# HIPS/DESI-MCMC

Hardware: AMD Instinct MI355X
Metric: source-pixel evals/sec + full-field log-lik ms, 10k sources x 5 bands x 2048^2 (higher is better)
Workload: dtype f64

## Files before the change

desi-mcmc_amd/csrc/k_render_hw.h:

```cpp
#pragma once
#include "k_render.h"

#ifdef CEL_ABLATE
#define CEL_ABLATE_BITS(flags) ((flags) >> 8)
#else
#define CEL_ABLATE_BITS(flags) 0
#endif

#define HW_TW 32
#define HW_TH 64
#ifdef HW_SYNC_BARRIER
#define HW_WAVE_SYNC() __syncthreads()
#else
#define HW_WAVE_SYNC()                                              \
    do {                                                            \
        __builtin_amdgcn_fence(__ATOMIC_ACQ_REL, "wavefront");      \
        __builtin_amdgcn_wave_barrier();                            \
    } while (0)
#endif
#define HW_PAD 12
#ifndef HW_PART_ENTRIES
#define HW_PART_ENTRIES 12
#endif

__host__ __device__ inline double quad_max_rect_hw(double a, double b, double c, double x1, double x2, double y1, double y2) {
    double m = a * x1 * x1 + (2.0 * b * x1 + c * y1) * y1;
    m = fmax(m, a * x2 * x2 + (2.0 * b * x2 + c * y1) * y1);
    m = fmax(m, a * x1 * x1 + (2.0 * b * x1 + c * y2) * y2);
    m = fmax(m, a * x2 * x2 + (2.0 * b * x2 + c * y2) * y2);
    return m * 1.00001;
}

template <int G, int STRIDE = HW_TW, bool SUM = false>
__device__ inline void rec_group_hw(const CompTab &T, const double *__restrict__ et, int k0, double x,
                                    int Y0, int ra, int rb, int L, bool on, double *__restrict__ acc_col,
                                    double *__restrict__ msum = nullptr) {
    double g[G], r[G], q[G];
    const double aon = on ? 1.0 : 0.0;
    for (int sa = ra; sa < rb; sa += L) {
        const int sb = min(sa + L, rb);
        const double y0 = (double)(Y0 + sa);
#pragma unroll
        for (int i = 0; i < G; i++) {
            const int k = k0 + i;
            double dx = x - T.mx[k], dy = y0 - T.my[k];
            double qb = T.qb[k], qc = T.qc[k];
            double hx = qb * dx + qc * dy;
            double e = -0.5 * (T.qa[k] * dx * dx + (qb * dx + hx) * dy);
            double er = fmin(fmax(-(hx + 0.5 * qc), -REC_EMAX * EXP_SCALE), REC_EMAX * EXP_SCALE);
            g[i] = (T.A[k] * aon) * exp_tab64(e, et);
            r[i] = exp_tab64(er, et);
            q[i] = T.eq[k];
        }
        int row = sa;
        for (; row + 1 < sb; row += 2) {
#pragma clang fp contract(off)
            double s0 = g[0], s1, g1[G], r1[G];
#pragma unroll
            for (int i = 1; i < G; i++) s0 += g[i];
#pragma unroll
            for (int i = 0; i < G; i++) {
                g1[i] = g[i] * r[i];
                r1[i] = r[i] * q[i];
            }
            s1 = g1[0];
#pragma unroll
            for (int i = 1; i < G; i++) s1 += g1[i];
#pragma unroll
            for (int i = 0; i < G; i++) {
                g[i] = g1[i] * r1[i];
                r[i] = r1[i] * q[i];
            }
            if (SUM) { *msum += s0; *msum += s1; }
            else {
                lds_add(&acc_col[row * STRIDE], s0);
                lds_add(&acc_col[(row + 1) * STRIDE], s1);
            }
        }
        if (row < sb) {
            double s0 = g[0];
#pragma unroll
            for (int i = 1; i < G; i++) s0 += g[i];
            if (SUM) *msum += s0;
            else lds_add(&acc_col[row * STRIDE], s0);
        }
    }
}

template <int N, int NT>
__device__ __forceinline__ void rec_walk_n(double (&g)[NT], double (&r)[NT], const double (&q)[NT], int row, int rend, bool advance,
                                           double *__restrict__ acc_col) {
    for (; row + 1 < rend; row += 2) {
#pragma clang fp contract(off)
        double s0 = g[0], s1, g1[N], r1[N];
#pragma unroll
        for (int i = 1; i < N; i++) s0 += g[i];
#pragma unroll
        for (int i = 0; i < N; i++) {
            g1[i] = g[i] * r[i];
            r1[i] = r[i] * q[i];
        }
        s1 = g1[0];
#pragma unroll
        for (int i = 1; i < N; i++) s1 += g1[i];
#pragma unroll
        for (int i = 0; i < N; i++) {
            g[i] = g1[i] * r1[i];
            r[i] = r1[i] * q[i];
        }
        lds_add(&acc_col[row * HW_TW], s0);
        lds_add(&acc_col[(row + 1) * HW_TW], s1);
    }
    if (row < rend) {
#pragma clang fp contract(off)
        double s0 = g[0];
#pragma unroll
        for (int i = 1; i < N; i++) s0 += g[i];
        lds_add(&acc_col[row * HW_TW], s0);
        if (advance) {
#pragma unroll
            for (int i = 0; i < N; i++) {
                g[i] = g[i] * r[i];
                r[i] = r[i] * q[i];
            }
        }
    }
}

template <int NB, int NS>
__device__ inline void rec_group_nested(const CompTab &T, const double *__restrict__ et, int kb, int ks, double x, int Y0,
                                        int ga, int gb, int sa, int sb, bool on, double *__restrict__ acc_col) {
    constexpr int NT = NB + NS;
    double g[NT], r[NT], q[NT];
    const double aon = on ? 1.0 : 0.0;
    auto seed = [&](int i, int k, double y0) {
        double dx = x - T.mx[k], dy = y0 - T.my[k];
        double qb = T.qb[k], qc = T.qc[k];
        double hx = qb * dx + qc * dy;
        double e = -0.5 * (T.qa[k] * dx * dx + (qb * dx + hx) * dy);
        double er = fmin(fmax(-(hx + 0.5 * qc), -REC_EMAX * EXP_SCALE), REC_EMAX * EXP_SCALE);
        g[i] = (T.A[k] * aon) * exp_tab64(e, et);
        r[i] = exp_tab64(er, et);
        q[i] = T.eq[k];
    };
#pragma unroll
    for (int i = 0; i < NB; i++) seed(i, kb + i, (double)(Y0 + ga));
    rec_walk_n<NB, NT>(g, r, q, ga, sa, true, acc_col);
#pragma unroll
    for (int i = 0; i < NS; i++) seed(NB + i, ks + i, (double)(Y0 + sa));
    rec_walk_n<NT, NT>(g, r, q, sa, sb, true, acc_col);
    rec_walk_n<NB, NT>(g, r, q, sb, gb, false, acc_col);
}

__host__ __device__ inline int nested_big(int gA) { return gA >= 5 ? 3 : (gA == 4 ? 2 : gA); }

template <int SHIFT = 3>
__device__ __forceinline__ int slot_by_rows(bool keep, int rlo, int rhi) {
    const int cls = keep ? 7 - min((rhi - rlo - 1) >> SHIFT, 7) : 8;
    int slot = 0, base = 0;
#pragma unroll
    for (int q = 0; q < 8; q++) {
        const unsigned long long bq = __ballot(cls == q);
        const int within = __builtin_amdgcn_mbcnt_hi((unsigned)(bq >> 32), __builtin_amdgcn_mbcnt_lo((unsigned)bq, 0));
        if (cls == q) slot = base + within;
        base += __popcll(bq);
    }
    return slot;
}

struct StarTab {
    double px[64], py[64], scale[64];
    int4 box[64];
    int cum[64];
    double qa[K_PSF], qb[K_PSF], qc[K_PSF], eq[K_PSF], A0[K_PSF], mux[K_PSF], muy[K_PSF];
};
static_assert(sizeof(StarTab) <= sizeof(CompTab), "the star table must fit the component table's storage");
#define STAR_EMAX 600.0


__device__ __forceinline__ bool star_setup(StarTab &ST, const BandDev *__restrict__ bd, const double *__restrict__ et, int lane) {
    bool bad = false;
    if (lane < K_PSF) {
        const double cxx = bd->cxx[lane], cxy = bd->cxy[lane], cyy = bd->cyy[lane];
        const double inv = 1.0 / (cxx * cyy - cxy * cxy);
        const double qa = cyy * inv, qb = -cxy * inv, qc = cxx * inv;
        ST.qa[lane] = qa * EXP_SCALE; ST.qb[lane] = qb * EXP_SCALE; ST.qc[lane] = qc * EXP_SCALE;
        ST.eq[lane] = exp_tab64(-qc * EXP_SCALE, et);
        ST.A0[lane] = bd->w[lane] * (0.5 / PI_D) * sqrt(inv);
        ST.mux[lane] = bd->mux[lane]; ST.muy[lane] = bd->muy[lane];
        const double rb_ = bd->R + 2.0;
        const double emax = 0.5 * quad_max_rect_hw(qa, qb, qc, -rb_ - bd->mux[lane], rb_ - bd->mux[lane],
                                                   -rb_ - bd->muy[lane], rb_ - bd->muy[lane]);
        bad = !(emax <= STAR_EMAX);
    }
    const bool ok = (__ballot(bad) == 0ull);
    __syncthreads();
    return ok;
}

__device__ __forceinline__ void star_stage(const RenderArgs &a, StarTab &ST, const SrcRec *__restrict__ recs, int64_t off, int base, int nb,
                                           int lane, int X0, int Y0, int strict, int lfirst = 0, int lstride = 1 ) {
    __syncthreads();
    double2 pp = make_double2(0.0, 0.0);
    double sc = 0.0;
    int4 bx4 = make_int4(0, 0, 0, 0);
    int nrows = -1;
    if (lane < nb) {
        const SrcRec *rp = recs + a.lists[off + lfirst + (int64_t)lstride * (base + lane)];
        pp = *reinterpret_cast<const double2 *>(&rp->px);
        sc = rp->scale;
        bx4 = *reinterpret_cast<const int4 *>(&rp->x0);
        nrows = max(min(bx4.w, Y0 + HW_TH) - max(bx4.z + strict, Y0), 0);
        const int ncols = max(min(bx4.y, X0 + HW_TW) - max(bx4.x + strict, X0), 0);
        if (ncols == 0) nrows = 0;
    }
    int *srows = reinterpret_cast<int *>(ST.scale);
    srows[lane] = nrows;
    __syncthreads();
    int rank = 0;
    for (int j = 0; j < nb; j++) {
        const int rj = srows[j];
        rank += (rj > nrows || (rj == nrows && j < lane)) ? 1 : 0;
    }
    __syncthreads();
    if (lane < nb) {
        ST.px[rank] = pp.x; ST.py[rank] = pp.y; ST.scale[rank] = sc;
        ST.box[rank] = bx4;
    }
    __syncthreads();
}

template <bool DIAG, int CW>
__device__ __forceinline__ void star_walk(const RenderArgs &a, StarTab &ST, const double *__restrict__ et, double *__restrict__ acc,
                                          int nb, int lane, int Xa, int Y0, int strict, unsigned &dbg_halfrows,
                                          unsigned char *__restrict__ own = nullptr) {
    double cqa[K_PSF], cqb[K_PSF], cqc[K_PSF], ceq[K_PSF], cA0[K_PSF], cmx[K_PSF], cmy[K_PSF];
#pragma unroll
    for (int k = 0; k < K_PSF; k++) {
        cqa[k] = ST.qa[k]; cqb[k] = ST.qb[k]; cqc[k] = ST.qc[k]; ceq[k] = ST.eq[k];
        cA0[k] = ST.A0[k]; cmx[k] = ST.mux[k]; cmy[k] = ST.muy[k];
    }
    const int dbg = DIAG ? CEL_ABLATE_BITS(a.flags) : 0;
    int w = 0;
    if (lane < nb) {
        const int4 q = ST.box[lane];
        const int nr = max(min(q.w, Y0 + HW_TH) - max(q.z + strict, Y0), 0);
        w = (nr > 0) ? max(min(q.y, Xa + CW) - max(q.x + strict, Xa), 0) : 0;
    }
    int incl = w;
#pragma unroll
    for (int o = 1; o < 64; o <<= 1) {
        const int up = __shfl_up(incl, o);
        if (lane >= o) incl += up;
    }
    const int total = __builtin_amdgcn_readlane(incl, 63);
    ST.cum[lane] = (lane < nb) ? incl - w : 0x3fffffff;
    if (own) {
#pragma unroll
        for (int cidx = 0; cidx < CW; cidx++)
            if (cidx < w) own[incl - w + cidx] = (unsigned char)lane;
    }
    __syncthreads();
    for (int t0 = 0; t0 < total && !(dbg & 2); t0 += 64) {
        const int t = t0 + lane;
        const bool valid = t < total;
        int j = 0;
        if (own) {
            j = own[min(t, total - 1)];
        } else {
#pragma unroll
            for (int step = 32; step > 0; step >>= 1)
                if (ST.cum[min(j + step, 63)] <= t && j + step < 64) j += step;
        }
        const double px = ST.px[j], py = ST.py[j];
        const int4 bx = ST.box[j];
        const int bx0 = max(bx.x + strict, Xa), by0 = bx.z + strict;
        const int xi = bx0 + (t - ST.cum[j]);
        const int ra = max(by0, Y0) - Y0;
        const int n = (valid && !(dbg & 1)) ? max(min(bx.w, Y0 + HW_TH) - Y0 - ra, 0) : 0;
        const double amp = valid ? ST.scale[j] : 0.0;
        const int nmax = __builtin_amdgcn_readlane(n, 0);
        if (DIAG && a.timing) dbg_halfrows += 2u * (unsigned)nmax * K_PSF;
        const double x = (double)xi;
        double g[K_PSF], r[K_PSF];
        const double y0 = (double)(Y0 + ra);
#pragma unroll
        for (int k = 0; k < K_PSF; k++) {
            const double dx = x - (px + cmx[k]), dy = y0 - (py + cmy[k]);
            const double hx = cqb[k] * dx + cqc[k] * dy;
            const double e = -0.5 * (cqa[k] * dx * dx + (cqb[k] * dx + hx) * dy);
            const double er = fmin(fmax(-(hx + 0.5 * cqc[k]), -REC_EMAX * EXP_SCALE), REC_EMAX * EXP_SCALE);
            g[k] = (cA0[k] * amp) * exp_tab64(e, et);
            r[k] = exp_tab64(er, et);
        }
        double *rowp = acc + ra * CW + (valid ? xi - Xa : 0);
        int i = 0;
        for (; i + 3 < nmax; i += 4, rowp += 4 * CW) {
#pragma clang fp contract(off)
            double g1[K_PSF], r1[K_PSF];
            const double s0 = (g[0] + g[1]) + g[2];
#pragma unroll
            for (int k = 0; k < K_PSF; k++) { g1[k] = g[k] * r[k]; r1[k] = r[k] * ceq[k]; }
            const double s1 = (g1[0] + g1[1]) + g1[2];
#pragma unroll
            for (int k = 0; k < K_PSF; k++) { g[k] = g1[k] * r1[k]; r[k] = r1[k] * ceq[k]; }
            const double s2 = (g[0] + g[1]) + g[2];
#pragma unroll
            for (int k = 0; k < K_PSF; k++) { g1[k] = g[k] * r[k]; r1[k] = r[k] * ceq[k]; }
            const double s3 = (g1[0] + g1[1]) + g1[2];
#pragma unroll
            for (int k = 0; k < K_PSF; k++) { g[k] = g1[k] * r1[k]; r[k] = r1[k] * ceq[k]; }
            if (i + 3 < n) {
                lds_add(&rowp[0], s0);
                lds_add(&rowp[CW], s1);
                lds_add(&rowp[2 * CW], s2);
                lds_add(&rowp[3 * CW], s3);
            } else {
                if (i < n) lds_add(&rowp[0], s0);
                if (i + 1 < n) lds_add(&rowp[CW], s1);
                if (i + 2 < n) lds_add(&rowp[2 * CW], s2);
            }
        }
        for (; i < nmax; i++, rowp += CW) {
#pragma clang fp contract(off)
            if (i < n) lds_add(&rowp[0], (g[0] + g[1]) + g[2]);
#pragma unroll
            for (int k = 0; k < K_PSF; k++) { g[k] = g[k] * r[k]; r[k] = r[k] * ceq[k]; }
        }
    }
}

template <bool DIAG>
__device__ __forceinline__ void star_pass(const RenderArgs &a, StarTab &ST, const double *__restrict__ et, double *__restrict__ acc,
                                          const SrcRec *__restrict__ recs, int64_t off, int nstar, int lane, int X0, int Y0,
                                          int strict, unsigned &dbg_halfrows, unsigned &dbg_pairs, int lfirst = 0, int lstride = 1) {
    for (int base = 0; base < nstar; base += 64) {
        const int nb = min(64, nstar - base);
        star_stage(a, ST, recs, off, base, nb, lane, X0, Y0, strict, lfirst, lstride);
        if (DIAG && a.timing) { dbg_pairs += (unsigned)nb; }
        star_walk<DIAG, HW_TW>(a, ST, et, acc, nb, lane, X0, Y0, strict, dbg_halfrows);
    }
}


template <bool PRE, bool DIAG = false>
__device__ __forceinline__ void hw_epilogue(const RenderArgs &a, const double *__restrict__ acc, double *__restrict__ lt,
                                            const BandDev *__restrict__ bd, int tile, int b, int xi, int Y0, int lane,
                                            const double *ne_pre) {
    const int half = lane >> 5;
    __syncthreads();
    lt[lane] = c_log_ic[lane];
    lt[64 + lane] = c_log_lc[lane];
    __syncthreads();
    const double eps = bd->eps;
    const bool store = !(a.flags & CEL_RENDER_NO_STORE);
    const bool ll = (a.flags & CEL_RENDER_LOGLIK) != 0;
    double part = 0.0;
    const int64_t plane = (int64_t)b * a.H * a.W;
    const int dbg = DIAG ? CEL_ABLATE_BITS(a.flags) : 0;
    const bool inside = (xi - (lane & 31) + HW_TW <= a.W) && (Y0 + HW_TH <= a.H);
    if (inside && ll && !PRE && !dbg) {
        const int64_t base = plane + (int64_t)(Y0 + half) * a.W + xi;
        double ne[HW_TH / 2];
#pragma unroll
        for (int r = 0; r < HW_TH / 2; r++) ne[r] = a.nelec[base + (int64_t)(2 * r) * a.W];
        if (store) {
#pragma unroll
            for (int r = 0; r < HW_TH / 2; r++) {
                const double lam = eps + acc[r * 64 + lane];
                a.lambda[base + (int64_t)(2 * r) * a.W] = lam;
                part += ne[r] * log_tab(lam, lt) - lam;
            }
        } else {
#pragma unroll
            for (int r = 0; r < HW_TH / 2; r++) {
                const double lam = eps + acc[r * 64 + lane];
                part += ne[r] * log_tab(lam, lt) - lam;
            }
        }
    } else if (inside && !ll && !dbg) {
        if (store) {
            const int64_t base = plane + (int64_t)(Y0 + half) * a.W + xi;
#pragma unroll
            for (int r = 0; r < HW_TH / 2; r++) a.lambda[base + (int64_t)(2 * r) * a.W] = eps + acc[r * 64 + lane];
        }
    } else if (xi < a.W && !(dbg & 16)) {
        const int64_t base = plane + (int64_t)(Y0 + half) * a.W + xi;
        double ne[HW_TH / 2];
#pragma unroll
        for (int r = 0; r < HW_TH / 2; r++)
            ne[r] = PRE ? ne_pre[r] : ((ll && Y0 + 2 * r + half < a.H) ? a.nelec[base + (int64_t)(2 * r) * a.W] : 0.0);
#pragma unroll
        for (int r = 0; r < HW_TH / 2; r++) {
            if (Y0 + 2 * r + half < a.H) {
                double lam = eps + acc[r * 64 + lane];
                if (store) a.lambda[base + (int64_t)(2 * r) * a.W] = lam;
                if (ll) part += (dbg & 4) ? ne[r] - lam : ne[r] * log_tab(lam, lt) - lam;
            }
        }
    }
    if (ll) {
        part = wave_sum(part);
        if (lane == 0) a.partials[tile] = part;
    }
}

__device__ __forceinline__ void hw_empty_tile(const RenderArgs &a, const BandDev *__restrict__ bd, int tile, int b, int X0, int Y0,
                                              int lane, unsigned long long t_start) {
    const int half = lane >> 5, xi = X0 + (lane & 31);
    const double eps = bd->eps;
    const bool store = !(a.flags & CEL_RENDER_NO_STORE);
    const bool ll = (a.flags & CEL_RENDER_LOGLIK) != 0;
    const int64_t base = (int64_t)b * a.H * a.W + (int64_t)(Y0 + half) * a.W + xi;
    double part = 0.0;
    if ((a.W & 31) == 0 && Y0 + HW_TH <= a.H) {
        const int cp = lane & 15, rq = lane >> 4;
        const int64_t b2 = (int64_t)b * a.H * a.W + (int64_t)(Y0 + rq) * a.W + X0 + 2 * cp;
        const double leps = ll ? log(eps) : 0.0;
        double2 ne2[HW_TH / 4];
        if (ll) {
#pragma unroll
            for (int r = 0; r < HW_TH / 4; r++)
                ne2[r] = *reinterpret_cast<const double2 *>(a.nelec + b2 + (int64_t)(4 * r) * a.W);
        }
#pragma unroll
        for (int r = 0; r < HW_TH / 4; r++) {
            if (store) *reinterpret_cast<double2 *>(a.lambda + b2 + (int64_t)(4 * r) * a.W) = make_double2(eps, eps);
            if (ll) part += (ne2[r].x * leps - eps) + (ne2[r].y * leps - eps);
        }
    } else if (xi < a.W) {
        double ne[HW_TH / 2];
#pragma unroll
        for (int r = 0; r < HW_TH / 2; r++)
            ne[r] = (ll && Y0 + 2 * r + half < a.H) ? a.nelec[base + (int64_t)(2 * r) * a.W] : 0.0;
        const double leps = ll ? log(eps) : 0.0;
#pragma unroll
        for (int r = 0; r < HW_TH / 2; r++) {
            if (Y0 + 2 * r + half < a.H) {
                if (store) a.lambda[base + (int64_t)(2 * r) * a.W] = eps;
                if (ll) part += ne[r] * leps - eps;
            }
        }
    }
    if (ll) {
        part = wave_sum(part);
        if (lane == 0) a.partials[tile] = part;
    }
    if (a.cost && lane == 0) a.cost[tile] = (int)min(wall_clock64() - t_start, 0x3fffffffull) + 1;
}

static_assert(sizeof(CompTab) >= 128 * sizeof(double), "log table must fit the component table");
template <bool DIAG, int PARTS = 1>
__global__ void __launch_bounds__(64)
k_render_hw(RenderArgs a) {
    __shared__ double acc[HW_TH * HW_TW];
    __shared__ CompTab T;
    __shared__ double et[64];
    const int lane = threadIdx.x;
    const int half = lane >> 5, col = lane & 31;
    unsigned long long *const timing = DIAG ? a.timing : nullptr;
    const int dbg = DIAG ? CEL_ABLATE_BITS(a.flags) : 0;
    const unsigned long long t_start = (timing || a.cost) ? wall_clock64() : 0ull;
    int tpos = blockIdx.x, part = 0;
    if (PARTS > 1) {
        const int q = blockIdx.x >> 3;
        tpos = (q / PARTS) * 8 + (blockIdx.x & 7);
        part = q % PARTS;
        if (tpos >= a.B * a.ntx * a.nty) return;
    }
    const int tile = a.order ? a.order[tpos] : tpos;
    if (PARTS == 1 && !DIAG && a.dirty && !a.dirty[tile]) return;
    const int per_band = a.ntx * a.nty;
    const int b = tile / per_band;
    const int t = tile - b * per_band;
    const int ty = t / a.ntx, tx = t - ty * a.ntx;
    const int X0 = tx * HW_TW, Y0 = ty * HW_TH;
    const int xi = X0 + col;
    const double x = (double)xi;
    const BandDev *bd = a.bands + b;

    const int cnt = a.tile_cnt[tile];
    if (dbg & 8) return;
    if (cnt == 0 && !timing) {
        if (part == 0) hw_empty_tile(a, bd, tile, b, X0, Y0, lane, t_start);
        return;
    }
    const int peff = (PARTS > 1) ? min(PARTS, max(1, (cnt + HW_PART_ENTRIES - 1) / HW_PART_ENTRIES)) : 1;
    if (PARTS > 1 && part >= peff) return;

    et[lane] = exp2((double)lane * (1.0 / 64.0));
#pragma unroll
    for (int r = 0; r < HW_TH / 2; r++) acc[r * 64 + lane] = 0.0;

    const int64_t off = a.tile_off[tile];
    const SrcRec *recs = a.recs + (int64_t)b * a.S;
    const double Tdrop = a.tail_T;
    const double eps_sky = bd->eps;
    const bool dropping = (a.variant != 0) && (Tdrop > 0.0) && (eps_sky > 0.0);
    const float log_eps = dropping ? __logf((float)eps_sky) : 0.0f;
    const int strict = (a.flags >> 2) & 1;

    unsigned dbg_pairrows = 0, dbg_comprows = 0, dbg_pairs = 0;
    float dbg_area = 0.f;
    unsigned dbg_halfrows = 0;
    const int nent_all = (int)min((int64_t)cnt, a.capacity > off ? a.capacity - off : (int64_t)0);
    int nstar = min(a.tile_nstar ? a.tile_nstar[tile] : 0, nent_all);
    if (dbg & 32) nstar = 0;
    if (a.variant == 0) nstar = 0;
    if (nstar > 0) {
        StarTab &ST = *reinterpret_cast<StarTab *>(&T);
        __syncthreads();
        if (!star_setup(ST, bd, et, lane)) nstar = 0;
    }
    const int nstar_all = nstar;
    if (PARTS > 1) nstar = (nstar > part) ? (nstar - part + peff - 1) / peff : 0;
    if (nstar > 0)
        star_pass<DIAG>(a, *reinterpret_cast<StarTab *>(&T), et, acc, recs, off, nstar, lane, X0, Y0, strict, dbg_halfrows, dbg_pairs,
                        PARTS > 1 ? part : 0, peff);

    const LaneConst lc = lane_consts(lane, bd);
    const int64_t off2 = off + nstar_all + (PARTS > 1 ? part : 0);
    int nent = (dbg & 32) ? 0 : nent_all - nstar_all;
    if (PARTS > 1) nent = (nent > part) ? (nent - part + peff - 1) / peff : 0;
    int idx64 = (lane < nent) ? a.lists[off2 + (int64_t)peff * lane] : 0;
    int recw_next = (nent > 0) ? rec_fetch(recs, __builtin_amdgcn_readlane(idx64, 0), lane) : 0;

    for (int e = 0; e < nent; e++) {
        const int recw = recw_next;
        if (e + 1 < nent) {
            if (((e + 1) & 63) == 0) idx64 = (e + 1 + lane < nent) ? a.lists[off2 + (int64_t)peff * (e + 1 + lane)] : 0;
            recw_next = rec_fetch(recs, __builtin_amdgcn_readlane(idx64, (e + 1) & 63), lane);
        }
        const RecU rec = rec_unpack(recw);
        const RecU *rp = &rec;
        const int type = rec.type;
        const int K = (type == 0) ? K_PSF : K_GAL;
        const int bx0 = rp->x0 + strict, bx1 = rp->x1, by0 = rp->y0 + strict, by1 = rp->y1;
        const int ra = max(by0, Y0) - Y0, rb = min(by1, Y0 + HW_TH) - Y0;
        const bool on = (xi >= bx0) && (xi < bx1);
        const double xa = (double)max(bx0, X0), xb = (double)(min(bx1, X0 + HW_TW) - 1);
        const double ya = (double)(Y0 + ra), yb = (double)(Y0 + rb - 1);

        bool keep = false;
        Comp c;
        int Lk = 0, rlo = ra, rhi = rb;
        if (lane < K) {
            c = make_comp_lc(lc, rec);
            double Tk = dropping ? Tdrop + (double)(__logf((float)fabs(c.A)) - log_eps) : 100.0;
            if (dropping) {
                double qmin = quad_min_rect(c.qa, c.qb, c.qc, xa - c.mx, xb - c.mx, ya - c.my, yb - c.my);
                keep = (0.5 * qmin <= Tk);
                float ylo, yhi;
                quad_rows_on_columns(c.qa, c.qb, c.qc, 2.0 * fmax(Tk, 0.0), xa - c.mx, xb - c.mx, ylo, yhi);
                const float cy = (float)(c.my - (double)Y0);
                rlo = max(ra, (int)ceilf(cy + ylo - 0.02f));
                rhi = min(rb, (int)floorf(cy + yhi + 0.02f) + 1);
                keep = keep && (rhi > rlo);
            } else {
                keep = true;
            }
            Lk = seg_len(c.qc, fmin(fmax(Tk, 1.0), 300.0));
        }
        const unsigned long long km = __ballot(keep);
        const int Kk = __popcll(km);
        if (timing) {
            int ir = keep ? rhi - rlo : 0;
            float cw = 0.f;
            if (keep) {
                double Tk2 = Tdrop + (double)__logf((float)(fabs(c.A) / eps_sky));
                float hx = sqrt_f32(2.0f * (float)fmax(Tk2, 0.0) / (float)c.ixx) + 1.0f;
                float lo = fmaxf((float)xa, (float)c.mx - hx), hi = fminf((float)xb + 1.f, (float)c.mx + hx);
                cw = fmaxf(hi - lo, 0.f);
            }
            float ar = (float)ir * cw;
            for (int o = 32; o; o >>= 1) { ir += __shfl_xor(ir, o); ar += __shfl_xor(ar, o); }
            dbg_pairrows += (unsigned)ir; dbg_area += ar;
        }
        HW_WAVE_SYNC();
        if (lane < 4) { T.gL[lane] = 4096; T.gr0[lane] = HW_TH; T.gr1[lane] = 0; T.gs0[lane] = HW_TH; T.gs1[lane] = 0; }
        const int slot = slot_by_rows(keep, rlo, rhi);
        if (keep) {
            const int p = slot;
            T.A[p] = c.A; T.mx[p] = c.mx; T.my[p] = c.my;
            T.qa[p] = c.qa * EXP_SCALE; T.qb[p] = c.qb * EXP_SCALE; T.qc[p] = c.qc * EXP_SCALE;
            T.eq[p] = exp_tab64(-c.qc * EXP_SCALE, et);
            const int gi = p / (2 * REC_G);
            atomicMin(&T.gL[gi], Lk);
            atomicMin(&T.gr0[gi], rlo);
            atomicMax(&T.gr1[gi], rhi);
            const int Rp = min(2 * REC_G, Kk - gi * (2 * REC_G));
            if (p - gi * (2 * REC_G) >= 2 * nested_big((Rp + 1) / 2)) {
                atomicMin(&T.gs0[gi], rlo);
                atomicMax(&T.gs1[gi], rhi);
            }
        }
        if (lane < HW_PAD) {
            int p = Kk + lane;
            T.A[p] = 0.0; T.mx[p] = 0.0; T.my[p] = 0.0;
            T.qa[p] = 0.0; T.qb[p] = 0.0; T.qc[p] = 0.0;
            T.eq[p] = 1.0;
        }
        HW_WAVE_SYNC();
        if (a.variant == 0) {
            const int kh = (Kk + 1) / 2;
            const int k0 = half ? kh : 0, k1 = half ? Kk : kh;
            for (int row = ra; row < rb; row++) {
                double v = eval_direct(T, k0, k1, x, (double)(Y0 + row), 1.0 / EXP_SCALE);
                if (on) lds_add(&acc[row * HW_TW + col], v);
            }
            continue;
        }
        for (int p0 = 0; p0 < Kk; p0 += 2 * REC_G) {
            const int R = min(2 * REC_G, Kk - p0);
            const int gA = (R + 1) / 2;
            const int gi = p0 / (2 * REC_G);
            const int L = __builtin_amdgcn_readfirstlane(T.gL[gi]);
            const int ga = __builtin_amdgcn_readfirstlane(T.gr0[gi]);
            const int gb = __builtin_amdgcn_readfirstlane(T.gr1[gi]);
            const int k0 = half ? p0 + gA : p0;
            const int nb = nested_big(gA);
            const bool nested = (gA >= 4) && (gb - ga <= L);
            int sa = 0, sb = 0;
            if (nested) {
                sa = __builtin_amdgcn_readfirstlane(T.gs0[gi]);
                sb = __builtin_amdgcn_readfirstlane(T.gs1[gi]);
                sa = min(max(sa, ga), gb);
                sb = max(min(sb, gb), sa);
            }
            if (timing) {
                dbg_comprows += nested ? (unsigned)(gb - ga) * (unsigned)(2 * nb) + (unsigned)(sb - sa) * (unsigned)(R - 2 * nb)
                                       : (unsigned)(gb - ga) * (unsigned)R;
                dbg_pairs += 1;
            }
            if (nested) {
                double *colp = acc + col;
                const int kb = p0 + half * nb, ks = p0 + 2 * nb + half * (gA - nb);
                switch (gA) {
                case 6: rec_group_nested<3, 3>(T, et, kb, ks, x, Y0, ga, gb, sa, sb, on, colp); break;
                case 5: rec_group_nested<3, 2>(T, et, kb, ks, x, Y0, ga, gb, sa, sb, on, colp); break;
                default: rec_group_nested<2, 2>(T, et, kb, ks, x, Y0, ga, gb, sa, sb, on, colp); break;
                }
                continue;
            }
            if (L < 4) {
                const int k1 = half ? p0 + R : p0 + gA;
                for (int row = ga; row < gb; row++) {
                    double v = eval_direct(T, k0, k1, x, (double)(Y0 + row), 1.0 / EXP_SCALE);
                    if (on) lds_add(&acc[row * HW_TW + col], v);
                }
                continue;
            }
            double *colp = acc + col;
            switch (gA) {
            case 6: rec_group_hw<6>(T, et, k0, x, Y0, ga, gb, L, on, colp); break;
            case 5: rec_group_hw<5>(T, et, k0, x, Y0, ga, gb, L, on, colp); break;
            case 4: rec_group_hw<4>(T, et, k0, x, Y0, ga, gb, L, on, colp); break;
            case 3: rec_group_hw<3>(T, et, k0, x, Y0, ga, gb, L, on, colp); break;
            case 2: rec_group_hw<2>(T, et, k0, x, Y0, ga, gb, L, on, colp); break;
            default: rec_group_hw<1>(T, et, k0, x, Y0, ga, gb, L, on, colp); break;
            }
        }
    }

    if (PARTS > 1 && peff > 1) {
        __syncthreads();
        double *slab = a.slabs + ((size_t)tile * PARTS + part) * (HW_TH * HW_TW);
#pragma unroll
        for (int r = 0; r < HW_TH / 2; r++) slab[r * 64 + lane] = acc[r * 64 + lane];
        asm volatile("s_waitcnt vmcnt(0)" ::: "memory");
        __syncthreads();
        int ticket = 0;
        if (lane == 0) {
            __builtin_amdgcn_fence(__ATOMIC_RELEASE, "agent");
            asm volatile("s_waitcnt vmcnt(0)" ::: "memory");
            ticket = __hip_atomic_fetch_add(&a.part_cnt[tile], 1, __ATOMIC_RELAXED, __HIP_MEMORY_SCOPE_AGENT);
        }
        ticket = __builtin_amdgcn_readfirstlane(ticket);
        if (ticket != peff - 1) return;
        if (lane == 0) {
            __hip_atomic_store(&a.part_cnt[tile], 0, __ATOMIC_RELAXED, __HIP_MEMORY_SCOPE_AGENT);
            __builtin_amdgcn_fence(__ATOMIC_ACQUIRE, "agent");
            asm volatile("s_waitcnt vmcnt(0)" ::: "memory");
        }
        __syncthreads();
        const double *s0 = a.slabs + (size_t)tile * PARTS * (HW_TH * HW_TW);
#pragma unroll 4
        for (int r = 0; r < HW_TH / 2; r++) {
            double v = s0[r * 64 + lane];
            for (int p = 1; p < peff; p++) v += s0[(size_t)p * (HW_TH * HW_TW) + r * 64 + lane];
            acc[r * 64 + lane] = v;
        }
    }
    hw_epilogue<false, DIAG>(a, acc, reinterpret_cast<double *>(&T), bd, tile, b, xi, Y0, lane, nullptr);
    if (a.cost && lane == 0) a.cost[tile] = (int)min((wall_clock64() - t_start) * (unsigned long long)peff, 0x3fffffffull) + 1;
    if (timing && lane == 0) {
        timing[3 * (size_t)tile + 0] = t_start;
        timing[3 * (size_t)tile + 1] = wall_clock64();
        timing[3 * (size_t)tile + 2] = (unsigned long long)(unsigned)cnt | ((unsigned long long)dbg_pairs << 12) |
                                               ((unsigned long long)(dbg_comprows + dbg_halfrows) << 32);
        if ((a.flags >> 8) & 128)
            timing[3 * (size_t)tile + 2] = (unsigned long long)dbg_pairrows | ((unsigned long long)(unsigned)(dbg_area / 32.f) << 32);
    }
}
```

Measured before the change: 355.9 billion.

## Add multi-row stepped Gaussian recurrence walk for long column segments

Adds a multi-row recurrence ('mw') that precomputes per-component ratio powers, so each step emits M rows (2 or 4) and advances the Gaussian by M rows at once. This breaks the serial one-multiply-per-row dependency chain and exposes more independent FMAs per step. It is used when the segment length is at least 16, for both the plain and the nested component groups. To bound the compounded ratio powers it tightens the exponent clamp to a quarter of the old range, at some cost in extra registers and possible rounding drift.

Measured after the change: 364.8 billion (median of 6 runs). 2.5% higher.

```diff
diff --git a/desi-mcmc_amd/csrc/k_render_hw.h b/desi-mcmc_amd/csrc/k_render_hw.h
--- a/desi-mcmc_amd/csrc/k_render_hw.h
+++ b/desi-mcmc_amd/csrc/k_render_hw.h
@@ -150,6 +150,126 @@
     for (int i = 0; i < NS; i++) seed(NB + i, ks + i, (double)(Y0 + sa));
     rec_walk_n<NT, NT>(g, r, q, sa, sb, true, acc_col);
     rec_walk_n<NB, NT>(g, r, q, sb, gb, false, acc_col);
+}
+
+#define MW_LMIN 16
+#define MW_EMAX (REC_EMAX / 4.0)
+#define MW_LONG 40
+
+template <int M>
+__device__ __forceinline__ void mw_build(double r, double q, double (&P)[4], double (&c)[4]) {
+    double t = r;
+    P[0] = r;
+#pragma unroll
+    for (int j = 1; j < M; j++) {
+        t = t * q;
+        P[j] = P[j - 1] * t;
+    }
+    double qm = q;
+#pragma unroll
+    for (int s = 1; s < M; s <<= 1) qm = qm * qm;
+    c[0] = qm;
+#pragma unroll
+    for (int j = 1; j < M; j++) c[j] = c[j - 1] * qm;
+}
+
+template <int N, int M, int NT, bool KEEP = false, typename KQ>
+__device__ __forceinline__ void mw_walk(const CompTab &T, double (&g)[NT], double (&P)[NT][4], const double (&c)[NT][4], KQ kq,
+                                        int row, int rend, bool advance, double *__restrict__ acc_col) {
+    for (; row + M <= rend; row += M) {
+#pragma clang fp contract(off)
+        double s[M];
+        s[0] = g[0];
+#pragma unroll
+        for (int i = 1; i < N; i++) s[0] += g[i];
+#pragma unroll
+        for (int j = 1; j < M; j++) {
+            s[j] = g[0] * P[0][j - 1];
+#pragma unroll
+            for (int i = 1; i < N; i++) s[j] = fma(g[i], P[i][j - 1], s[j]);
+        }
+#pragma unroll
+        for (int i = 0; i < N; i++) {
+            g[i] = g[i] * P[i][M - 1];
+#pragma unroll
+            for (int j = 0; j < M; j++) P[i][j] = P[i][j] * c[i][j];
+        }
+#pragma unroll
+        for (int j = 0; j < M; j++) lds_add(&acc_col[(row + j) * HW_TW], s[j]);
+    }
+    if (row < rend) {
+        double q[N];
+#pragma unroll
+        for (int i = 0; i < N; i++) q[i] = T.eq[kq(i)];
+        for (; row < rend; row++) {
+#pragma clang fp contract(off)
+            double s0 = g[0];
+#pragma unroll
+            for (int i = 1; i < N; i++) s0 += g[i];
+            lds_add(&acc_col[row * HW_TW], s0);
+            if (row + 1 < rend || advance) {
+#pragma unroll
+                for (int i = 0; i < N; i++) {
+                    g[i] = g[i] * P[i][0];
+                    P[i][0] = P[i][0] * q[i];
+                    if (KEEP) P[i][1] = P[i][1] * c[i][0];
+                }
+            }
+        }
+    }
+}
+
+__device__ __forceinline__ void mw_seed(const CompTab &T, const double *__restrict__ et, int k, double x, double y0, double aon,
+                                        double &g, double &r) {
+    double dx = x - T.mx[k], dy = y0 - T.my[k];
+    double qb = T.qb[k], qc = T.qc[k];
+    double hx = qb * dx + qc * dy;
+    double e = -0.5 * (T.qa[k] * dx * dx + (qb * dx + hx) * dy);
+    double er = fmin(fmax(-(hx + 0.5 * qc), -MW_EMAX * EXP_SCALE), MW_EMAX * EXP_SCALE);
+    g = (T.A[k] * aon) * exp_tab64(e, et);
+    r = exp_tab64(er, et);
+}
+
+template <int G, int M>
+__device__ inline void rec_group_mw(const CompTab &T, const double *__restrict__ et, int k0, double x,
+                                    int Y0, int ra, int rb, int L, bool on, double *__restrict__ acc_col) {
+    double g[G], P[G][4], c[G][4];
+    const double aon = on ? 1.0 : 0.0;
+    auto kq = [k0](int i) { return k0 + i; };
+    for (int sa = ra; sa < rb; sa += L) {
+        const int sb = min(sa + L, rb);
+#pragma unroll
+        for (int i = 0; i < G; i++) {
+            double r;
+            mw_seed(T, et, k0 + i, x, (double)(Y0 + sa), aon, g[i], r);
+            mw_build<M>(r, T.eq[k0 + i], P[i], c[i]);
+        }
+        mw_walk<G, M, G>(T, g, P, c, kq, sa, sb, false, acc_col);
+    }
+}
+
+template <int NB, int NS>
+__device__ inline void rec_group_nested_mw(const CompTab &T, const double *__restrict__ et, int kb, int ks, double x, int Y0,
+                                           int ga, int gb, int sa, int sb, bool on, double *__restrict__ acc_col) {
+    constexpr int NT = NB + NS;
+    double g[NT], P[NT][4], c[NT][4];
+    const double aon = on ? 1.0 : 0.0;
+    auto kq = [kb, ks](int i) { return i < NB ? kb + i : ks + (i - NB); };
+#pragma unroll
+    for (int i = 0; i < NB; i++) {
+        double r;
+        mw_seed(T, et, kb + i, x, (double)(Y0 + ga), aon, g[i], r);
+        mw_build<2>(r, T.eq[kb + i], P[i], c[i]);
+    }
+    mw_walk<NB, 2, NT, true>(T, g, P, c, kq, ga, sa, true, acc_col);
+#pragma unroll
+    for (int i = NB; i < NT; i++) {
+        double r;
+        mw_seed(T, et, ks + (i - NB), x, (double)(Y0 + sa), aon, g[i], r);
+        mw_build<2>(r, T.eq[ks + (i - NB)], P[i], c[i]);
+    }
+    mw_walk<NT, 2, NT, true>(T, g, P, c, kq, sa, sb, true, acc_col);
+    mw_walk<NB, 2, NT>(T, g, P, c, kq, sb, gb, false, acc_col);
 }
 
 __host__ __device__ inline int nested_big(int gA) { return gA >= 5 ? 3 : (gA == 4 ? 2 : gA); }
@@ -635,6 +755,14 @@
             if (nested) {
                 double *colp = acc + col;
                 const int kb = p0 + half * nb, ks = p0 + 2 * nb + half * (gA - nb);
+                if (L >= MW_LMIN) {
+                    switch (gA) {
+                    case 6: rec_group_nested_mw<3, 3>(T, et, kb, ks, x, Y0, ga, gb, sa, sb, on, colp); break;
+                    case 5: rec_group_nested_mw<3, 2>(T, et, kb, ks, x, Y0, ga, gb, sa, sb, on, colp); break;
+                    default: rec_group_nested_mw<2, 2>(T, et, kb, ks, x, Y0, ga, gb, sa, sb, on, colp); break;
+                    }
+                    continue;
+                }
                 switch (gA) {
                 case 6: rec_group_nested<3, 3>(T, et, kb, ks, x, Y0, ga, gb, sa, sb, on, colp); break;
                 case 5: rec_group_nested<3, 2>(T, et, kb, ks, x, Y0, ga, gb, sa, sb, on, colp); break;
@@ -651,6 +779,23 @@
                 continue;
             }
             double *colp = acc + col;
+            if (L >= MW_LMIN) {
+                switch (gA) {
+                case 6: rec_group_mw<6, 2>(T, et, k0, x, Y0, ga, gb, L, on, colp); break;
+                case 5: rec_group_mw<5, 2>(T, et, k0, x, Y0, ga, gb, L, on, colp); break;
+                case 4: rec_group_mw<4, 2>(T, et, k0, x, Y0, ga, gb, L, on, colp); break;
+                case 3: if (min(L, gb - ga) >= MW_LONG) rec_group_mw<3, 4>(T, et, k0, x, Y0, ga, gb, L, on, colp);
+                        else rec_group_mw<3, 2>(T, et, k0, x, Y0, ga, gb, L, on, colp);
+                        break;
+                case 2: if (min(L, gb - ga) >= MW_LONG) rec_group_mw<2, 4>(T, et, k0, x, Y0, ga, gb, L, on, colp);
+                        else rec_group_mw<2, 2>(T, et, k0, x, Y0, ga, gb, L, on, colp);
+                        break;
+                default: if (min(L, gb - ga) >= MW_LONG) rec_group_mw<1, 4>(T, et, k0, x, Y0, ga, gb, L, on, colp);
+                         else rec_group_mw<1, 2>(T, et, k0, x, Y0, ga, gb, L, on, colp);
+                         break;
+                }
+                continue;
+            }
             switch (gA) {
             case 6: rec_group_hw<6>(T, et, k0, x, Y0, ga, gb, L, on, colp); break;
             case 5: rec_group_hw<5>(T, et, k0, x, Y0, ga, gb, L, on, colp); break;
```
